# cornellius-gp/linear_operator

Measured on AMD Instinct MI355X. Metric: cg_member_matvecs_per_sec, higher is better.
Workload: dtype f32

## Files before the change

linear_operator_amd/csrc/lo_rspace3.hip:

```cpp
#include <algorithm>
#include <atomic>
#include <mutex>
#include <type_traits>
#include <stdlib.h>

#include "lo_device.h"
#include "lo_internal.h"
#include "lo_cg_onchip.h"
#include "lo_group_reduce.h"
#include "lo_cg_close.h"
#include "lo_f64_lanes.h"

namespace lo {

namespace {

typedef float f32x4 __attribute__((ext_vector_type(4)));
typedef __attribute__((address_space(1))) const f32x4 g_cf4;
typedef __attribute__((address_space(1))) const float g_cf;
typedef __attribute__((address_space(1))) float g_f;
typedef __attribute__((address_space(1))) const char g_cc;
template <class T>
__device__ __forceinline__ T* opaque_uniform(T* p) {
  asm volatile("" : "+s"(p));
  return p;
}

constexpr int R3_TPB = 256;
constexpr int R3_ROWS = 1024;

struct PeerOut {
  float* buf[7];
  int n;
  long long member_off;
};
PeerOut g_peer_out = {{nullptr, nullptr, nullptr, nullptr, nullptr, nullptr, nullptr}, 0, 0};
std::mutex g_peer_mu;

__host__ __device__ constexpr int r3_np(int RC) { return 2 * RC + 6; }

__device__ __forceinline__ unsigned xor4_dpp_u(unsigned x) {
  const int a = __builtin_amdgcn_update_dpp(0, (int)x, 0x104, 0xf, 0x5, false);
  return (unsigned)__builtin_amdgcn_update_dpp(a, (int)x, 0x114, 0xf, 0xa, false);
}
__device__ __forceinline__ double halve4_d(double lo, double hi, int lane) {
  const bool up = (lane & 4) != 0;
  const double keep = up ? hi : lo;
  const double send = up ? lo : hi;
  return keep + mk_d(xor4_dpp_u(lo_w(send)), xor4_dpp_u(hi_w(send)));
}

template <int CH>
__device__ __forceinline__ double rows_reduce_d(double (&p)[CH], int lane) {
  if constexpr (CH == 8) {
#pragma unroll
    for (int m = 0; m < 4; ++m) p[m] = halve4_d(p[m], p[m + 4], lane);
    p[0] = halve_pair_d<2>(p[0], p[2], lane);
    p[1] = halve_pair_d<2>(p[1], p[3], lane);
    return halve_pair_d<1>(p[0], p[1], lane);
  } else if constexpr (CH == 4) {
    p[0] = halve_pair_d<2>(p[0], p[2], lane);
    p[1] = halve_pair_d<2>(p[1], p[3], lane);
    return halve_pair_d<1>(p[0], p[1], lane);
  } else {
    return halve_pair_d<1>(p[0], p[1], lane);
  }
}

template <int RC, int GW>
__global__ __launch_bounds__(R3_TPB, 2) void k_cg_rspace3(OnchipArgs a, PeerOut po) {
  constexpr int CH = RC / 4;
  constexpr int RPI = 64 / CH;
  constexpr int NI = 256 / RPI;
  constexpr int NP = r3_np(RC);
  constexpr int MLD = RC + 2;
  constexpr int NH = RC / 2;
  constexpr int NG = 2 * GW * NP;
  __shared__ __attribute__((aligned(16))) float bst[4][256];
  __shared__ __attribute__((aligned(16))) float dst[4][256];
  __shared__ __attribute__((aligned(16))) double mat_s[3 * RC * MLD];
  __shared__ __attribute__((aligned(16))) double red[4][NP];
  __shared__ __attribute__((aligned(16))) double res[NP];
  __shared__ __attribute__((aligned(16))) double gv[4][32];
  __shared__ unsigned polw[GW > 1 ? NG : 2];
  const GroupPlace gp = group_place(GW, (int)gridDim.x / 8);
  if (!gp.active) return;
  const int grp = gp.grp, wig = gp.wig, ngroups = gp.ngroups;
  const int t = threadIdx.x, lane = t & 63, wave = t >> 6;
  const int wave_u = __builtin_amdgcn_readfirstlane(wave);
  unsigned long long* const gbase = a.gbuf + (size_t)grp * 2 * NG;
  unsigned tag = a.tag_base;
  bool same_xcd = false;
  const unsigned xcc = xcc_id();
  bool first = true;
  const int row0 = wig * R3_ROWS + 256 * wave_u;
  const int row0c = max(0, min(row0, a.N - 256));
  const bool di_full = a.dinv_mode == LO_DIAG_FULL;
  float* const bw = bst[wave_u];
  float* const dw = dst[wave_u];
  constexpr int NPF = 8;
  f32x4 pre[NPF];
  constexpr int NXT = NI - NPF;
  f32x4 nxt[NXT > 0 ? NXT : 1];
  auto request = [&](int64_t bm, int tl_, int i_lo, auto cnt, f32x4* dst) {
    const int ln_ = tl_ & 63, k_ = ln_ & (CH - 1), g_ = ln_ / CH;
    const unsigned loff = (unsigned)((g_ * RC + 4 * k_) * sizeof(float));
    g_cc* Cw = (g_cc*)(a.C + ((size_t)bm * a.N + row0c) * RC);
#pragma unroll
    for (int q = 0; q < decltype(cnt)::value / 8; ++q) {
      g_cc* bq = opaque_uniform(Cw + (i_lo + 8 * q + 4) * 1024);
#pragma unroll
      for (int i = 0; i < 8; ++i) dst[8 * q + i] = *(g_cf4*)(bq + loff + (i - 4) * 1024);
    }
  };
  int64_t b = grp;
  {
    int tl0 = t;
    asm volatile("" : "+v"(tl0));
    if (b < a.B) {
      request(b, tl0, 0, std::integral_constant<int, NPF>{}, pre);
      request(b, tl0, NPF, std::integral_constant<int, NXT>{}, nxt);
    } else {
#pragma unroll
      for (int i = 0; i < NPF; ++i) pre[i] = (f32x4){0.f, 0.f, 0.f, 0.f};
    }
  }
  while (b < a.B) {
    const bool stamp = a.dbg && b == a.dbg_member && wig == 0 && t == 0;
    if (stamp) a.dbg[0] = wall_clock64();
    int drawn = 0;
    if (wig == 0 && t == 0) drawn = atomicAdd(a.next_member, 1);
    int tl = t;
    asm volatile("" : "+v"(tl));
    const int ln = tl & 63, k = ln & (CH - 1), g = ln / CH;
    f32x4 Cr[NI];
#pragma unroll
    for (int i = 0; i < NPF; ++i) Cr[i] = pre[i];
#pragma unroll
    for (int i = 0; i < NXT; ++i) Cr[NPF + i] = nxt[i];
    float bq4[4], dq4[4];
    {
      g_cf* bb_ = opaque_uniform((g_cf*)(a.rhs + (size_t)b * a.N + row0c));
      g_cf* dd_ = opaque_uniform((g_cf*)(di_full ? a.dinv + (size_t)b * a.N + row0c : a.dinv + b));
      const int lo_e = row0 - row0c, hi_e = max(0, min(256, a.N - row0c));
      const int dstride = di_full ? 1 : 0;
#pragma unroll
      for (int m = 0; m < 4; ++m) {
        const int e = ln + 64 * m;
        const bool own = e >= lo_e && e < hi_e;
        bq4[m] = own ? bb_[e] : 0.f;
        dq4[m] = own ? dd_[e * dstride] : 0.f;
      }
    }
    constexpr int NM = (3 * RC * RC / 2 + R3_TPB - 1) / R3_TPB;
    f32x4 mv[NM];
    {
      typedef __attribute__((address_space(1))) const f32x4 g_m4;
      const g_m4* src = (const g_m4*)(a.RSD + (size_t)b * 6 * RC * RC);
#pragma unroll
      for (int u = 0; u < NM; ++u) {
        const int e = min(tl + R3_TPB * u, 3 * RC * RC / 2 - 1);
        const int ms = e / (RC * RC / 2);
        const int mg = ms == 0 ? 0 : ms + 1;
        mv[u] = src[(size_t)mg * (RC * RC / 2) + (e - ms * (RC * RC / 2))];
      }
    }
    const double lam_mine = a.RSD[((size_t)b * 6 + 5) * RC * RC + min(ln & 31, RC - 1)];
#pragma unroll
    for (int m = 0; m < 4; ++m) {
      bw[ln + 64 * m] = bq4[m];
      dw[ln + 64 * m] = dq4[m];
    }
#pragma unroll
    for (int u = 0; u < NM; ++u) {
      const int e = tl + R3_TPB * u;
      if (e < 3 * RC * RC / 2) {
        const int mi = e / (RC / 2), jj = e % (RC / 2);
        *reinterpret_cast<f32x4*>(&mat_s[mi * MLD + 2 * jj]) = mv[u];
      }
    }
    __builtin_amdgcn_wave_barrier();
    if (stamp) a.dbg[1] = wall_clock64();

    {
      double aw[4] = {0.0, 0.0, 0.0, 0.0}, au[4] = {0.0, 0.0, 0.0, 0.0};
#pragma unroll
      for (int i0 = 0; i0 < NI; i0 += 4) {
#pragma unroll
        for (int i = i0; i < i0 + 4; ++i) {
          const int r = RPI * i + g;
          const double bb = (double)bw[r];
          const double bd = bb * (double)dw[r];
          const double c0 = (double)Cr[i].x, c1 = (double)Cr[i].y, c2 = (double)Cr[i].z, c3 = (double)Cr[i].w;
          aw[0] = fma(c0, bd, aw[0]); au[0] = fma(c0, bb, au[0]);
          aw[1] = fma(c1, bd, aw[1]); au[1] = fma(c1, bb, au[1]);
          aw[2] = fma(c2, bd, aw[2]); au[2] = fma(c2, bb, au[2]);
          aw[3] = fma(c3, bd, aw[3]); au[3] = fma(c3, bb, au[3]);
        }
        __builtin_amdgcn_sched_barrier(0);
      }
      double s_acc = 0.0, a_acc = 0.0, d2_acc = 0.0;
#pragma unroll
      for (int j = 0; j < 4; ++j) {
        const int rw = 64 * j + RPI * k + g;
        const double bb = (double)bw[rw], di = (double)dw[rw];
        s_acc = fma(bb, bb * di, s_acc);
        a_acc = fma(bb, bb, a_acc);
        d2_acc = fma(di, di, d2_acc);
      }
      double h0 = halve_pair_d<32>(aw[0], au[0], ln), h1 = halve_pair_d<32>(aw[1], au[1], ln);
      double h2 = halve_pair_d<32>(aw[2], au[2], ln), h3 = halve_pair_d<32>(aw[3], au[3], ln);
      h0 = halve_pair_d<16>(h0, h2, ln);
      h1 = halve_pair_d<16>(h1, h3, ln);
      double mine = halve_pair_d<8>(h0, h1, ln);
      if constexpr (CH <= 4) mine = bfly_add_d<4>(mine);
      if constexpr (CH <= 2) mine = bfly_add_d<2>(mine);
      const int comp = (((ln >> 4) & 1) << 1) | ((ln >> 3) & 1);
      const bool writer = (ln & 7 & ~(CH - 1)) == 0;
      if (writer) red[wave_u][((ln >> 5) ? RC : 0) + 4 * k + comp] = mine;
      const double ssum = wave_sum_fast_d(s_acc), asum = wave_sum_fast_d(a_acc), d2sum = wave_sum_fast_d(d2_acc);
      if (ln == 0) {
        red[wave_u][2 * RC] = ssum;
        red[wave_u][2 * RC + 1] = asum;
        red[wave_u][2 * RC + 2] = (wig == 0 && wave_u == 0) ? (double)(ngroups + drawn) : 0.0;
        red[wave_u][2 * RC + 3] = d2sum;
        unsigned xc = xcc;
        asm volatile("" : "+s"(xc));
        red[wave_u][2 * RC + 4] = (first && wave_u == 0) ? (double)xc : 0.0;
        red[wave_u][2 * RC + 5] = (first && wave_u == 0) ? (double)(xc * xc) : 0.0;
      }
    }
#pragma unroll
    for (int i = 0; i < NI; ++i) asm volatile("" : "+v"(Cr[i]));
    __builtin_amdgcn_sched_barrier(0);
    if (a.prefetch & 4) __builtin_amdgcn_s_setprio(3);
    {
      ++tag;
      int tt = (int)threadIdx.x;
      asm volatile("" : "+v"(tt));
      __syncthreads();
      if constexpr (GW == 1) {
        if (tt < NP) res[tt] = (red[0][tt] + red[1][tt]) + (red[2][tt] + red[3][tt]);
      } else {
        unsigned long long* slot = gbase + (size_t)(tag & 1u) * NG;
        if (tt < NP) {
          const double v = (red[0][tt] + red[1][tt]) + (red[2][tt] + red[3][tt]);
          unsigned long long* mine = slot + ((size_t)wig * NP + tt) * 2;
          granule_store(mine, granule_pack_bits(tag, lo_w(v)), same_xcd);
          granule_store(mine + 1, granule_pack_bits(tag, hi_w(v)), same_xcd);
        }
        constexpr int PER = (NG + R3_TPB - 1) / R3_TPB;
        constexpr int CKQ = PER < 8 ? PER : 8;
        unsigned spin = 0;
        bool lost = false;
#pragma unroll 1
        for (int q0 = 0; q0 < PER && !lost; q0 += CKQ) {
          unsigned long long x[CKQ];
          for (;;) {
            bool ok = true;
#pragma unroll
            for (int q = 0; q < CKQ; ++q) {
              const int idx = tt + R3_TPB * (q0 + q);
              x[q] = granule_load(slot + min(idx, NG - 1));
              ok = ok && (granule_tag(x[q]) == tag);
            }
            if (ok) break;
            if (poll_give_up(spin, a.err)) {
              lost = true;
              break;
            }
            __builtin_amdgcn_s_sleep(1);
          }
#pragma unroll
          for (int q = 0; q < CKQ; ++q) {
            const int idx = tt + R3_TPB * (q0 + q);
            if (idx < NG) polw[idx] = granule_bits(x[q]);
          }
        }
        __syncthreads();
        if (tt < NP) {
          double tot = 0.0;
#pragma unroll
          for (int w = 0; w < GW; ++w) tot += mk_d(polw[(w * NP + tt) * 2], polw[(w * NP + tt) * 2 + 1]);
          res[tt] = tot;
        }
      }
      __syncthreads();
    }
    if (GW > 1 && first) {
      unsigned xc = xcc;
      asm volatile("" : "+s"(xc));
      same_xcd = same_xcd_verdict(res[2 * RC + 4], res[2 * RC + 5], GW, xc, a.allow_l2_handoff);
    }
    first = false;
    if (stamp) a.dbg[2] = wall_clock64();
    const int64_t b_next = (int64_t)res[2 * RC + 2];
    {
      int tp = t;
      asm volatile("" : "+v"(tp));
      if (b_next < a.B) {
        request(b_next, tp, 0, std::integral_constant<int, NPF>{}, pre);
      } else {
#pragma unroll
        for (int i = 0; i < NPF; ++i) pre[i] = (f32x4){0.f, 0.f, 0.f, 0.f};
      }
    }
    if (a.prefetch & 1) __builtin_amdgcn_s_setprio(3);

    const int j = lane & 31, hf = lane >> 5;
    const bool live = j < RC;
    const int jr = live ? j : RC - 1;
    double yj = 0.0, xi = 0.0;
    float nrm;
    {
      double a0 = res[2 * RC + 1], s = res[2 * RC];
      const double d2 = res[2 * RC + 3];
      nrm = sqrtf((float)a0);
      const bool rhs_zero = nrm < a.eps;
      if (rhs_zero) nrm = 1.0f;
      const double inv = 1.0 / (double)nrm;
      const double w0 = live ? res[jr] * inv : 0.0, u0 = live ? res[RC + jr] * inv : 0.0;
      s *= inv * inv;
      a0 *= inv * inv;
      float sa = a.stop_after;
      asm volatile("" : "+s"(sa));
      const double sure_rz = 2.0 * (double)sa * (double)sa * sqrt(d2);
      auto own_row_dot = [&](const double* mrow, const double* vec) {
        double a0_ = 0.0, a1_ = 0.0;
#pragma unroll
        for (int q = 0; q < NH; q += 2) {
          const double2 xa = *reinterpret_cast<const double2*>(mrow + q);
          const double2 xx = *reinterpret_cast<const double2*>(vec + q);
          a0_ = fma(xa.x, xx.x, a0_);
          a1_ = fma(xa.y, xx.y, a1_);
        }
        double lo_, up_;
        halves_d(a0_ + a1_, lo_, up_);
        return lo_ + up_;
      };
      double* myv = gv[wave];
      if (hf == 0) myv[j] = w0;
      __builtin_amdgcn_wave_barrier();
      const double* row0m = mat_s + (size_t)jr * MLD + hf * NH;
      double c0 = own_row_dot(row0m, myv + hf * NH);
      double e0 = own_row_dot(row0m + (size_t)1 * RC * MLD, myv + hf * NH);
      const double* nrow = row0m + (size_t)2 * RC * MLD;
      const double* tucol = mat_s + (size_t)(1 * RC + hf * NH) * MLD + jr;
      c0 = live ? c0 : 0.0;
      e0 = live ? e0 : 0.0;
      double tau2 = s - lanes32_sum_d(c0 * e0);
      tau2 = tau2 > 0.0 ? tau2 : 0.0;
      const bool delicate = !rhs_zero && tau2 < 1e-2 * s;
      const double lam = live ? lam_mine : 1.0;
      long long ts_a = 0, ts_b = 0;
      if (stamp) ts_a = wall_clock64();
      double cj = c0, qj = 0.0, etaj = 0.0;
      double cp = 1.0, qp = 0.0, etap = 0.0;
      double rz = 0.0, pApE = 0.0, alpha = 0.0, beta = 0.0;
      float rn = 0.f, last_alpha = 0.f;
      bool conv = false;
      unsigned close_flags = 0u;
      const size_t bc = (size_t)b;
      const bool rec = wig == 0 && lane == 0;
      const int last_owner = (a.iters - 1) & 3;
      for (int kk = -1; kk < a.iters; ++kk) {
        if (kk >= 0) {
          last_alpha = (float)alpha;
          etaj = fma(alpha, qj, etaj);
          etap = fma(alpha, qp, etap);
          cj = fma(-alpha * lam, qj, cj);
          cp = fma(-alpha, qp, cp);
        }
        const double lc = lam * cj;
        const bool lo_h = hf == 0;
        const float inv_rz = __builtin_amdgcn_rcpf((float)rz);
        const double red2 = row16_sum_d(halve_pair_d<16>(lo_h ? cj * cj : lc * qj, lo_h ? lc * cj : 0.0, lane));
        const auto pick = [&](double v, int ln_) {
          return mk_d((unsigned)__builtin_amdgcn_readlane((int)lo_w(v), ln_),
                      (unsigned)__builtin_amdgcn_readlane((int)hi_w(v), ln_));
        };
        const double cc = pick(red2, 0), clc = pick(red2, 16), clq = pick(red2, 32);
        const double rzn = fma(cp * cp, tau2, cc);
        const bool sure = rzn > sure_rz;
        const bool rec_first = kk == 0 && a.close_gran == nullptr && wave == 0;
        const bool rec_last = kk == a.iters - 1 && wave == last_owner;
        const bool own = rec_first || rec_last || !sure;
        float rnn = 0.f;
        if (kk < 0) {
          const float s1f = (float)a0;
          rnn = __builtin_amdgcn_sqrtf(s1f < 0.f ? 0.f : s1f);
        } else if (own) {
          const double dl = fma(-cp, c0, cj);
          __builtin_amdgcn_wave_barrier();
          if (hf == 0) myv[j] = dl;
          __builtin_amdgcn_wave_barrier();
          double gj_;
          {
            double a0_ = 0.0, a1_ = 0.0;
#pragma unroll
            for (int q = 0; q < NH; q += 2) {
              const double2 dd = *reinterpret_cast<const double2*>(myv + hf * NH + q);
              a0_ = fma(tucol[(size_t)q * MLD], dd.x, a0_);
              a1_ = fma(tucol[(size_t)(q + 1) * MLD], dd.y, a1_);
            }
            double lo_, up_;
            halves_d(a0_ + a1_, lo_, up_);
            gj_ = live ? lo_ + up_ : 0.0;
          }
          __builtin_amdgcn_wave_barrier();
          if (hf == 0) myv[j] = gj_;
          __builtin_amdgcn_wave_barrier();
          const double nd = own_row_dot(nrow, myv + hf * NH);
          const double r2 = row16_sum_d(halve_pair_d<16>(gj_ * nd, gj_ * u0, lane));
          const double dnd = pick(r2, 0), dm = pick(r2, 16);
          const double s1 = fma(cp, fma(cp, a0, 2.0 * dm), dnd);
          const float s1f = (float)s1;
          rnn = __builtin_amdgcn_sqrtf(s1f < 0.f ? 0.f : s1f);
        }
        if (kk >= 0) {
          beta = ((float)rz < a.eps) ? 0.0 : (double)((float)rzn * inv_rz);
          if (rhs_zero) rnn = 0.f;
          rn = rnn;
          if (rec && (rec_first || rec_last)) a.resid_rec[(size_t)kk * a.B + bc] = rn;
        } else {
          beta = 0.0;
          rn = rnn;
          if (wig == 0 && t == 0) a.init_conv[bc] = (rn < a.stop_after) ? 1 : 0;
          close_flags = ((rn < a.stop_after) ? 1u : 0u) | (delicate ? 4u : 0u);
          if (delicate && rec && wave == 0) atomicOr(a.err + 4, 1);
        }
        if (kk == 0 && (rnn != rnn || rzn != rzn)) close_flags |= 2u;
        conv = (own || rhs_zero) ? (rn < a.stop_after) : false;
        rz = rzn;
        pApE = fma(beta, fma(beta, pApE, 2.0 * clq), clc);
        qj = fma(beta, qj, cj);
        qp = fma(beta, qp, cp);
        const double pAp = fma(qp * qp, tau2, pApE);
        alpha = ((float)pAp < a.eps) ? 0.0 : (double)((float)rz * __builtin_amdgcn_rcpf((float)pAp));
        if (conv) alpha = 0.0;
      }
      if (stamp) ts_b = wall_clock64();
      if (rec && wave == last_owner) {
        a.rhs_norm[bc] = nrm;
        a.rhs_is_zero[bc] = rhs_zero ? 1 : 0;
        a.rz[bc] = (float)rz;
        a.alpha[bc] = last_alpha;
        a.beta[bc] = (float)beta;
        a.resid_norm[bc] = rn;
        a.has_conv[bc] = conv ? 1 : 0;
        if (a.close_gran) {
          granule_store(a.close_gran + b, granule_pack(a.close_epoch | close_flags, rn), false);
        }
      }
      __builtin_amdgcn_wave_barrier();
      if (hf == 0) myv[j] = fma(-etap, e0, etaj);
      __builtin_amdgcn_wave_barrier();
      xi = etap;
      {
        const double* col = mat_s + (size_t)(hf * NH) * MLD + jr;
        double a0_ = 0.0, a1_ = 0.0;
#pragma unroll
        for (int q = 0; q < NH; q += 2) {
          const double2 ee = *reinterpret_cast<const double2*>(myv + hf * NH + q);
          a0_ = fma(col[(size_t)q * MLD], ee.x, a0_);
          a1_ = fma(col[(size_t)(q + 1) * MLD], ee.y, a1_);
        }
        double lo_, up_;
        halves_d(a0_ + a1_, lo_, up_);
        yj = lo_ + up_;
      }
      yj = live ? yj : 0.0;
      if (stamp) {
        a.dbg[5] = ts_a - a.dbg[2];
        a.dbg[6] = ts_b - ts_a;
        a.dbg[7] = wall_clock64() - ts_b;
      }
      __builtin_amdgcn_wave_barrier();
      if (hf == 0) myv[j] = yj * (double)nrm;
      __builtin_amdgcn_wave_barrier();
    }
    if (!(a.prefetch & 2)) __builtin_amdgcn_s_setprio(0);
    if (stamp) a.dbg[3] = wall_clock64();
    {
      int l2 = lane;
      asm volatile("" : "+v"(l2));
      const int k2 = l2 & (CH - 1), g2 = l2 / CH;
      const double* myv = gv[wave];
      const double2 ya = *reinterpret_cast<const double2*>(&myv[4 * k2]);
      const double2 yb = *reinterpret_cast<const double2*>(&myv[4 * k2 + 2]);
      g_f* const xb = opaque_uniform((g_f*)(a.xout + (size_t)b * a.N + row0c));
      const bool more = b_next < a.B;
      g_cc* const Cn = (g_cc*)(a.C + ((size_t)(more ? b_next : b) * a.N + row0c) * RC);
      const unsigned loffn = (unsigned)((g2 * RC + 4 * k2) * sizeof(float));
#pragma unroll
      for (int js = 0; js < 4; ++js) {
        constexpr int J0 = NPF / CH;
        const int jj = (js + J0) & 3;
        double p[CH];
#pragma unroll
        for (int m = 0; m < CH; ++m) {
          const f32x4 c4 = Cr[CH * jj + m];
          p[m] = fma((double)c4.w, yb.y, fma((double)c4.z, yb.x, fma((double)c4.y, ya.y, (double)c4.x * ya.x)));
        }
        const double xv = rows_reduce_d<CH>(p, l2);
        const int rw = 64 * jj + RPI * k2 + g2;
        const int row = row0c + rw;
        const double acc = fma(xi, (double)bw[rw], xv);
        if (row >= row0 && row < a.N) {
          const float xval = (float)(acc * (double)dw[rw]);
          xb[rw] = xval;
          for (int pp = 0; pp < po.n; ++pp)
            ((g_f*)po.buf[pp])[((size_t)(b + po.member_off)) * a.N + row] = xval;
        }
        if (CH * jj >= NPF) {
          g_cc* bqn = opaque_uniform(Cn + (CH * jj + 4) * 1024);
#pragma unroll
          for (int m = 0; m < CH; ++m)
            nxt[CH * jj - NPF + m] = more ? *(g_cf4*)(bqn + loffn + (m - 4) * 1024) : (f32x4){0.f, 0.f, 0.f, 0.f};
        }
      }
      __builtin_amdgcn_wave_barrier();
    }
    __builtin_amdgcn_s_setprio(0);
    if (stamp) a.dbg[4] = wall_clock64();
    __syncthreads();
    b = b_next;
  }
  if (a.close_gran && wig == 0) cg_close_solve(a, ngroups, t);
}

int rspace3_prio() {
  static const int prio = [] {
    const char* e = getenv("LO_RS_PRIO");
    return e ? atoi(e) : 3;
  }();
  return prio;
}

constexpr size_t HO_MAX_WGS = 2 * 320;
constexpr size_t HO_GRAN_PER_WG = 432;
constexpr size_t HO_MAX_MEMBERS = 65536;
constexpr size_t HO_HEAD_BYTES = 256;
constexpr unsigned HO_TAG_LIMIT = 0xfff00000u;
constexpr unsigned HO_EPOCH_LIMIT = 0x1ffffff0u;
struct HandoffBlock {
  char* buf = nullptr;
  size_t bytes = 0;
  bool failed = false;
  unsigned next_tag = 1, next_epoch = 1;
  unsigned last_launch = 0;
  std::atomic<unsigned> confirmed{0};
  bool force_clear = false;
  unsigned clears = 0, launches = 0;
};
HandoffBlock g_handoff[16];
std::atomic<unsigned> g_handoff_ids{0};

HandoffBlock* handoff_block() {
  int dev = 0;
  if (hipGetDevice(&dev) != hipSuccess || dev < 0 || dev >= 16) return nullptr;
  HandoffBlock& h = g_handoff[dev];
  if (!h.buf && !h.failed) {
    h.bytes = HO_HEAD_BYTES + (HO_MAX_WGS * HO_GRAN_PER_WG + HO_MAX_MEMBERS) * sizeof(unsigned long long);
    if (hipMalloc(&h.buf, h.bytes) != hipSuccess || hipMemset(h.buf, 0, h.bytes) != hipSuccess) {
      (void)hipGetLastError();
      h.buf = nullptr;
      h.failed = true;
    }
  }
  return h.buf ? &h : nullptr;
}

bool handoff_advance(unsigned* next_tag, unsigned* next_epoch, int64_t B, unsigned* tag_base, unsigned* epoch) {
  bool wrap = false;
  const unsigned need = (unsigned)B + 2u;
  if (*next_tag >= HO_TAG_LIMIT - need || *next_epoch >= HO_EPOCH_LIMIT) {
    *next_tag = 1;
    *next_epoch = 1;
    wrap = true;
  }
  *tag_base = *next_tag;
  *epoch = *next_epoch;
  *next_tag += need;
  *next_epoch += 1;
  return wrap;
}

struct OwnedLaunch {
  bool inject;
  unsigned* launch_id;
};

template <int RC, int GW>
int rspace3_go(const OnchipArgs& a, int nwg, const OwnedLaunch* own, hipStream_t st) {
  int per_cu = 0;
  if (LO_OCCUPANCY_CACHED(per_cu, (k_cg_rspace3<RC, GW>), R3_TPB, 0) != hipSuccess || per_cu < 2) return LO_ERR_UNSUPPORTED;
  LO_PROF_BEGIN("cg_onchip", st);
  ResidentLaunch guard(st);
  OnchipArgs a2 = a;
  a2.prefetch = rspace3_prio();
  if (own) {
    hipStreamCaptureStatus cap = hipStreamCaptureStatusNone;
    if (hipStreamIsCapturing(st, &cap) != hipSuccess || cap != hipStreamCaptureStatusNone) {
      (void)hipGetLastError();
      return LO_ERR_UNSUPPORTED;
    }
    HandoffBlock* h = (a.B <= (int64_t)HO_MAX_MEMBERS && (size_t)2 * nwg <= HO_MAX_WGS) ? handoff_block() : nullptr;
    if (!h) return LO_ERR_UNSUPPORTED;
    bool clear = h->force_clear || h->last_launch != h->confirmed.load(std::memory_order_acquire);
    h->force_clear = false;
    clear = handoff_advance(&h->next_tag, &h->next_epoch, a.B, &a2.tag_base, &a2.close_epoch) || clear;
    h->last_launch = g_handoff_ids.fetch_add(1, std::memory_order_relaxed) + 1;
    if (h->last_launch == 0) h->last_launch = g_handoff_ids.fetch_add(1, std::memory_order_relaxed) + 1;
    *own->launch_id = h->last_launch;
    ++h->launches;
    if (clear) {
      ++h->clears;
      const int zrc = zero_span(h->buf, h->bytes, st);
      if (zrc) return zrc;
    }
    a2.close_epoch <<= 3;
    a2.handoff_owned = 1;
    a2.err = reinterpret_cast<int*>(h->buf);
    a2.next_member = a2.err + 1;
    a2.close_count = a2.err + 2;
    a2.gbuf = reinterpret_cast<unsigned long long*>(h->buf + HO_HEAD_BYTES);
    a2.close_gran = a2.gbuf + HO_MAX_WGS * HO_GRAN_PER_WG;
    if (own->inject) LO_HIP_CHECK(hipMemsetAsync(a2.err, 1, 1, st));
  }
  PeerOut po;
  {
    std::lock_guard<std::mutex> lk(g_peer_mu);
    po = g_peer_out;
  }
  hipLaunchKernelGGL((k_cg_rspace3<RC, GW>), dim3(2 * nwg), dim3(R3_TPB), 0, st, a2, po);
  LO_PROF_END(st);
  LO_LAUNCH_CHECK();
  return LO_OK;
}

template <int RC>
int rspace3_gw(const OnchipArgs& a, int nwg, const OwnedLaunch* own, hipStream_t st) {
  switch (a.GW) {
    case 1: return rspace3_go<RC, 1>(a, nwg, own, st);
    case 2: return rspace3_go<RC, 2>(a, nwg, own, st);
    case 4: return rspace3_go<RC, 4>(a, nwg, own, st);
    case 8: return rspace3_go<RC, 8>(a, nwg, own, st);
    case 16: return rspace3_go<RC, 16>(a, nwg, own, st);
    case 32: return rspace3_go<RC, 32>(a, nwg, own, st);
  }
  return LO_ERR_UNSUPPORTED;
}

int rspace3_dispatch(int RC, const OnchipArgs& a, int nwg, const OwnedLaunch* own, hipStream_t st) {
  if (!a.RSD || a.x || a.c != 1 || a.ab_rec || !a.xout || a.GW > 32 || a.N < 256 || (int64_t)a.GW * R3_ROWS < a.N)
    return LO_ERR_UNSUPPORTED;
  if (RC == 32) return rspace3_gw<32>(a, nwg, own, st);
  if (RC == 16) return rspace3_gw<16>(a, nwg, own, st);
  if (RC == 8) return rspace3_gw<8>(a, nwg, own, st);
  return LO_ERR_UNSUPPORTED;
}

}

int rspace3_launch(int RC, const OnchipArgs& a, int nwg, hipStream_t st) { return rspace3_dispatch(RC, a, nwg, nullptr, st); }

int rspace3_launch_owned(int RC, const OnchipArgs& a, int nwg, bool inject, unsigned* launch_id, hipStream_t st) {
  if (!a.close_gran || !a.close_ctrl || !a.close_mirror || a.dbg) return LO_ERR_UNSUPPORTED;
  const OwnedLaunch own = {inject, launch_id};
  return rspace3_dispatch(RC, a, nwg, &own, st);
}

void handoff_launch_confirm(unsigned launch_id) {
  int dev = 0;
  if (hipGetDevice(&dev) != hipSuccess || dev < 0 || dev >= 16) return;
  g_handoff[dev].confirmed.store(launch_id, std::memory_order_release);
}

}

extern "C" int lo_peer_gather_set(float* const* bufs, int n, long long member_offset) {
  if (n < 0 || n > 7 || (n > 0 && !bufs)) return LO_ERR_BADARG;
  std::lock_guard<std::mutex> lk(lo::g_peer_mu);
  for (int i = 0; i < 7; ++i) lo::g_peer_out.buf[i] = i < n ? bufs[i] : nullptr;
  lo::g_peer_out.n = n;
  lo::g_peer_out.member_off = member_offset;
  return LO_OK;
}

extern "C" int lo_resident_handoff_debug(int32_t force_clear, int64_t set_next_tag, int64_t set_next_epoch, uint32_t* out) {
  lo::ResidentLock guard;
  int dev = 0;
  if (hipGetDevice(&dev) != hipSuccess || dev < 0 || dev >= 16) return LO_ERR_BADARG;
  lo::HandoffBlock& h = lo::g_handoff[dev];
  if (set_next_tag > 0xffffffffll || set_next_epoch > 0xffffffffll) return LO_ERR_BADARG;
  if (set_next_tag >= 0) h.next_tag = (unsigned)set_next_tag;
  if (set_next_epoch >= 0) h.next_epoch = (unsigned)set_next_epoch;
  if (force_clear) h.force_clear = true;
  if (out) {
    out[0] = h.next_tag;
    out[1] = h.next_epoch;
    out[2] = h.clears;
    out[3] = h.launches;
  }
  return LO_OK;
}
```

Before: 34.96 million.

## Run the redundant per-member CG solve on a single rotating wave

Previously all four waves of each workgroup ran the same small CG recurrence redundantly, each with its own scratch vector. Now only one solver wave, rotating by member count, runs the solve and publishes the y vector and xi to shared memory, and a workgroup barrier is added before the back-projection. The idle waves are freed to issue the prefetch loads and to yield issue slots. The cost is an extra __syncthreads per member and the serialisation of the other waves behind the solver.

```diff
diff --git a/linear_operator_amd/csrc/lo_rspace3.hip b/linear_operator_amd/csrc/lo_rspace3.hip
--- a/linear_operator_amd/csrc/lo_rspace3.hip
+++ b/linear_operator_amd/csrc/lo_rspace3.hip
@@ -27,6 +27,12 @@
 }
 
 constexpr int R3_TPB = 256;
+#ifndef R3_SOLVER_WAVE
+#define R3_SOLVER_WAVE(taken) ((taken) & 3)
+#endif
+#ifndef R3_CHAIN_PRIO
+#define R3_CHAIN_PRIO 3
+#endif
 constexpr int R3_ROWS = 1024;
 
 struct PeerOut {
@@ -81,7 +87,8 @@
   __shared__ __attribute__((aligned(16))) double mat_s[3 * RC * MLD];
   __shared__ __attribute__((aligned(16))) double red[4][NP];
   __shared__ __attribute__((aligned(16))) double res[NP];
-  __shared__ __attribute__((aligned(16))) double gv[4][32];
+  __shared__ __attribute__((aligned(16))) double gvs[32];
+  __shared__ __attribute__((aligned(16))) double pub[32 + 2];
   __shared__ unsigned polw[GW > 1 ? NG : 2];
   const GroupPlace gp = group_place(GW, (int)gridDim.x / 8);
   if (!gp.active) return;
@@ -114,6 +121,7 @@
     }
   };
   int64_t b = grp;
+  int taken = 0;
   {
     int tl0 = t;
     asm volatile("" : "+v"(tl0));
@@ -293,7 +301,10 @@
       same_xcd = same_xcd_verdict(res[2 * RC + 4], res[2 * RC + 5], GW, xc, a.allow_l2_handoff);
     }
     first = false;
-    if (stamp) a.dbg[2] = wall_clock64();
+    const int solver = R3_SOLVER_WAVE(taken);
+    const bool solves = wave_u == solver;
+    const bool sstamp = a.dbg && b == a.dbg_member && wig == 0 && solves && lane == 0;
+    if (sstamp) a.dbg[2] = wall_clock64();
     const int64_t b_next = (int64_t)res[2 * RC + 2];
     {
       int tp = t;
@@ -305,14 +316,14 @@
         for (int i = 0; i < NPF; ++i) pre[i] = (f32x4){0.f, 0.f, 0.f, 0.f};
       }
     }
-    if (a.prefetch & 1) __builtin_amdgcn_s_setprio(3);
-
-    const int j = lane & 31, hf = lane >> 5;
-    const bool live = j < RC;
-    const int jr = live ? j : RC - 1;
-    double yj = 0.0, xi = 0.0;
-    float nrm;
-    {
+    if (a.prefetch & 1) __builtin_amdgcn_s_setprio(R3_CHAIN_PRIO);
+
+    if (solves) {
+      const int j = lane & 31, hf = lane >> 5;
+      const bool live = j < RC;
+      const int jr = live ? j : RC - 1;
+      double yj = 0.0, xi = 0.0;
+      float nrm;
       double a0 = res[2 * RC + 1], s = res[2 * RC];
       const double d2 = res[2 * RC + 3];
       nrm = sqrtf((float)a0);
@@ -338,7 +349,7 @@
         halves_d(a0_ + a1_, lo_, up_);
         return lo_ + up_;
       };
-      double* myv = gv[wave];
+      double* myv = gvs;
       if (hf == 0) myv[j] = w0;
       __builtin_amdgcn_wave_barrier();
       const double* row0m = mat_s + (size_t)jr * MLD + hf * NH;
@@ -353,7 +364,7 @@
       const bool delicate = !rhs_zero && tau2 < 1e-2 * s;
       const double lam = live ? lam_mine : 1.0;
       long long ts_a = 0, ts_b = 0;
-      if (stamp) ts_a = wall_clock64();
+      if (sstamp) ts_a = wall_clock64();
       double cj = c0, qj = 0.0, etaj = 0.0;
       double cp = 1.0, qp = 0.0, etap = 0.0;
       double rz = 0.0, pApE = 0.0, alpha = 0.0, beta = 0.0;
@@ -362,7 +373,6 @@
       unsigned close_flags = 0u;
       const size_t bc = (size_t)b;
       const bool rec = wig == 0 && lane == 0;
-      const int last_owner = (a.iters - 1) & 3;
       for (int kk = -1; kk < a.iters; ++kk) {
         if (kk >= 0) {
           last_alpha = (float)alpha;
@@ -382,8 +392,8 @@
         const double cc = pick(red2, 0), clc = pick(red2, 16), clq = pick(red2, 32);
         const double rzn = fma(cp * cp, tau2, cc);
         const bool sure = rzn > sure_rz;
-        const bool rec_first = kk == 0 && a.close_gran == nullptr && wave == 0;
-        const bool rec_last = kk == a.iters - 1 && wave == last_owner;
+        const bool rec_first = kk == 0 && a.close_gran == nullptr;
+        const bool rec_last = kk == a.iters - 1;
         const bool own = rec_first || rec_last || !sure;
         float rnn = 0.f;
         if (kk < 0) {
@@ -425,9 +435,9 @@
         } else {
           beta = 0.0;
           rn = rnn;
-          if (wig == 0 && t == 0) a.init_conv[bc] = (rn < a.stop_after) ? 1 : 0;
+          if (rec) a.init_conv[bc] = (rn < a.stop_after) ? 1 : 0;
           close_flags = ((rn < a.stop_after) ? 1u : 0u) | (delicate ? 4u : 0u);
-          if (delicate && rec && wave == 0) atomicOr(a.err + 4, 1);
+          if (delicate && rec) atomicOr(a.err + 4, 1);
         }
         if (kk == 0 && (rnn != rnn || rzn != rzn)) close_flags |= 2u;
         conv = (own || rhs_zero) ? (rn < a.stop_after) : false;
@@ -439,8 +449,8 @@
         alpha = ((float)pAp < a.eps) ? 0.0 : (double)((float)rz * __builtin_amdgcn_rcpf((float)pAp));
         if (conv) alpha = 0.0;
       }
-      if (stamp) ts_b = wall_clock64();
-      if (rec && wave == last_owner) {
+      if (sstamp) ts_b = wall_clock64();
+      if (rec) {
         a.rhs_norm[bc] = nrm;
         a.rhs_is_zero[bc] = rhs_zero ? 1 : 0;
         a.rz[bc] = (float)rz;
@@ -470,24 +480,24 @@
         yj = lo_ + up_;
       }
       yj = live ? yj : 0.0;
-      if (stamp) {
+      if (sstamp) {
         a.dbg[5] = ts_a - a.dbg[2];
         a.dbg[6] = ts_b - ts_a;
         a.dbg[7] = wall_clock64() - ts_b;
       }
-      __builtin_amdgcn_wave_barrier();
-      if (hf == 0) myv[j] = yj * (double)nrm;
-      __builtin_amdgcn_wave_barrier();
-    }
+      if (hf == 0) pub[j] = yj * (double)nrm;
+      if (lane == 0) pub[32] = xi;
+    }
+    __syncthreads();
     if (!(a.prefetch & 2)) __builtin_amdgcn_s_setprio(0);
-    if (stamp) a.dbg[3] = wall_clock64();
+    if (sstamp) a.dbg[3] = wall_clock64();
     {
       int l2 = lane;
       asm volatile("" : "+v"(l2));
       const int k2 = l2 & (CH - 1), g2 = l2 / CH;
-      const double* myv = gv[wave];
-      const double2 ya = *reinterpret_cast<const double2*>(&myv[4 * k2]);
-      const double2 yb = *reinterpret_cast<const double2*>(&myv[4 * k2 + 2]);
+      const double2 ya = *reinterpret_cast<const double2*>(&pub[4 * k2]);
+      const double2 yb = *reinterpret_cast<const double2*>(&pub[4 * k2 + 2]);
+      const double xi = pub[32];
       g_f* const xb = opaque_uniform((g_f*)(a.xout + (size_t)b * a.N + row0c));
       const bool more = b_next < a.B;
       g_cc* const Cn = (g_cc*)(a.C + ((size_t)(more ? b_next : b) * a.N + row0c) * RC);
@@ -525,6 +535,7 @@
     if (stamp) a.dbg[4] = wall_clock64();
     __syncthreads();
     b = b_next;
+    ++taken;
   }
   if (a.close_gran && wig == 0) cg_close_solve(a, ngroups, t);
 }
```

Result: slower. 32.59 million (-6.8%).
